# ahuang73/HemoCell

Hardware: AMD Instinct MI355X
Metric: MLUPS + cell-vertex updates/s, 256^3 pipeflow 10% Hct (higher is better)
Workload: dtype f64

## Files before the change

hemocell_amd/csrc/ibm.hip:

```cpp
#include "cells.h"
#include <type_traits>
#include <hipcub/hipcub.hpp>
#include <cstdlib>
#include <cstring>
#include <numeric>

namespace {

__global__ __launch_bounds__(256) void ibm_spread_kernel(LatView v, long n, const double *px, const double *py, const double *pz,
                                                         double *fx, double *fy, double *fz, const double *rx, const double *ry, const double *rz,
                                                         double *F, int limit_on, double f_limit, const int *vert_cell, const int *tag, const unsigned char *dead) {
  const long i = (long)blockIdx.x * 256 + threadIdx.x;
  if (i >= n) return;
  if (dead[i] || tag[vert_cell[i]] == 1) return;
  double f0 = fx[i], f1 = fy[i], f2 = fz[i];
  if (limit_on) {
    const double mag = sqrt((f0 * f0 + f1 * f1) + f2 * f2);
    if (mag > f_limit) {
      const double sc = f_limit / mag;
      f0 *= sc; f1 *= sc; f2 *= sc;
      fx[i] = f0; fy[i] = f1; fz[i] = f2;
    }
  }
  Stencil s;
  phi2_stencil(v, px[i], py[i], pz[i], s);
#pragma unroll
  for (int k = 0; k < 8; k++) {
    if (s.node[k] < 0) continue;
    v.dirty[s.node[k] >> 4] = v.epoch;
    double *Fn = F + 3 * s.node[k];
    unsafeAtomicAdd(Fn, ((rx ? rx[i] : 0.0) + f0) * s.w[k]);
    unsafeAtomicAdd(Fn + 1, ((ry ? ry[i] : 0.0) + f1) * s.w[k]);
    unsafeAtomicAdd(Fn + 2, ((rz ? rz[i] : 0.0) + f2) * s.w[k]);
  }
}

__global__ __launch_bounds__(256) void spread_emit_kernel(LatView v, int nv, long n, const int *order, long ebase, const double *px, const double *py,
                                                          const double *pz, double *fx, double *fy, double *fz, const double *rx, const double *ry,
                                                          const double *rz, int limit_on, double f_limit, const int *tag, const unsigned char *dead,
                                                          unsigned int *keys, int *vals, double *c0, double *c1, double *c2) {
  const long g = (long)blockIdx.x * 256 + threadIdx.x;
  if (g >= n) return;
  const int cell = order[g / nv];
  const long i = (long)cell * nv + (g % nv);
  const long e0 = (ebase + g) * 8;
  const bool live = tag[cell] != 1 && !dead[i];
  Stencil s;
  double f0 = 0.0, f1 = 0.0, f2 = 0.0;
  if (live) {
    f0 = fx[i]; f1 = fy[i]; f2 = fz[i];
    if (limit_on) {
      const double mag = sqrt((f0 * f0 + f1 * f1) + f2 * f2);
      if (mag > f_limit) { const double sc = f_limit / mag; f0 *= sc; f1 *= sc; f2 *= sc; fx[i] = f0; fy[i] = f1; fz[i] = f2; }
    }
    if (rx) { f0 = rx[i] + f0; f1 = ry[i] + f1; f2 = rz[i] + f2; }
    phi2_stencil(v, px[i], py[i], pz[i], s);
  }
#pragma unroll
  for (int k = 0; k < 8; k++) {
    const bool adm = live && s.node[k] >= 0;
    keys[e0 + k] = adm ? (unsigned int)s.node[k] : 0xffffffffu;
    vals[e0 + k] = (int)(e0 + k);
    c0[e0 + k] = adm ? f0 * s.w[k] : 0.0; c1[e0 + k] = adm ? f1 * s.w[k] : 0.0; c2[e0 + k] = adm ? f2 * s.w[k] : 0.0;
  }
}

__global__ __launch_bounds__(256) void spread_gather_kernel(LatView v, long n, const unsigned int *keys, const int *vals, const double *c0, const double *c1,
                                                            const double *c2, double *F) {
  const long s = (long)blockIdx.x * 256 + threadIdx.x;
  if (s >= n) return;
  const unsigned int key = keys[s];
  if (key == 0xffffffffu || (s > 0 && keys[s - 1] == key)) return;
  double a0 = 0.0, a1 = 0.0, a2 = 0.0;
  for (long q = s; q < n && keys[q] == key; q++) { const int e = vals[q]; a0 += c0[e]; a1 += c1[e]; a2 += c2[e]; }
  v.dirty[key >> 4] = v.epoch;
  double *Fn = F + 3 * (long)key;
  Fn[0] += a0; Fn[1] += a1; Fn[2] += a2;
}

struct PopView {
  const double *f; const double *F; double bx, by, bz; long qs;
  hc::BodyRegions reg;
};
struct OpenPopView : PopView { const int *ob_code; const double *ob_val; };
template <bool OPEN> using Pops = std::conditional_t<OPEN, OpenPopView, PopView>;

template <bool OPEN = false>
__device__ __forceinline__ void node_velocity(const LatView &v, const Pops<OPEN> &pv, int lx, int ly, int lz, long node, double u[3]) {
  if (v.halo_x && (lx <= -HALO || lx >= v.nx + HALO - 1)) { u[0] = u[1] = u[2] = 0.0; return; }
  if (v.halo_x && (lx == -1 || lx == v.nx)) {
    const double *hu = v.halo_u[lx < 0 ? 0 : 1];
    if (hu) { const long k = (long)ly * v.nz + lz; u[0] = hu[k]; u[1] = hu[v.ny_nz + k]; u[2] = hu[2L * v.ny_nz + k]; return; }
  }
  const hc::Nbr nb = hc::neighbours(v, v.plane, lx, ly, lz);
  double r = 0.0, jx = 0.0, jy = 0.0, jz = 0.0;
  [[maybe_unused]] double f[OPEN ? HC_Q : 1];
#define M(Q, CX, CY, CZ)                                                              \
  {                                                                                   \
    bool ok; const long off = hc::src_off<CX, CY, CZ>(nb, ok);                        \
    const double fq = ok ? pv.f[(long)Q * pv.qs + node + off] : 0.0;                 \
    if constexpr (OPEN) f[Q] = fq;                                                    \
    else {                                                                            \
      r += fq;                                                                        \
      if (CX == 1) jx += fq; else if (CX == -1) jx += -fq;                            \
      if (CY == 1) jy += fq; else if (CY == -1) jy += -fq;                            \
      if (CZ == 1) jz += fq; else if (CZ == -1) jz += -fq;                            \
    }                                                                                 \
  }
  FOR_Q(M)
#undef M
  if constexpr (OPEN) {
    if (v.mask[node] == 0) {
      const int code = pv.ob_code[node];
      if (code >= 0) hc::zou_he_node(f, code, pv.ob_val);
    }
    hc::moments(f, r, jx, jy, jz);
  }
  const double invRho = 1.0 / (1.0 + r);
  double bx = pv.bx, by = pv.by, bz = pv.bz;
  if (pv.reg.n) {
    int xg = v.x0 + lx;
    if (xg < 0) xg += v.nx_global; else if (xg >= v.nx_global) xg -= v.nx_global;
    region_force(pv.reg, xg, ly, lz, bx, by, bz);
  }
  u[0] = jx * invRho + (bx + pv.F[3 * node]) / 2.0;
  u[1] = jy * invRho + (by + pv.F[3 * node + 1]) / 2.0;
  u[2] = jz * invRho + (bz + pv.F[3 * node + 2]) / 2.0;
}

template <bool OPEN = false>
__global__ __launch_bounds__(256) void face_velocity_kernel(LatView v, Pops<OPEN> pv, int lx0, double *out0, int lx1, double *out1) {
  const int k = blockIdx.x * 256 + threadIdx.x;
  if (k >= v.ny_nz) return;
  const int lx = blockIdx.y ? lx1 : lx0;
  double *out = blockIdx.y ? out1 : out0;
  const int ly = k / v.nz, lz = k - ly * v.nz;
  const long node = (long)(lx + HALO) * v.plane + (long)ly * v.nz + lz;
  double u[3] = {0.0, 0.0, 0.0};
  if (v.mask[node] == 0) node_velocity<OPEN>(v, pv, lx, ly, lz, node, u);
  out[k] = u[0]; out[v.ny_nz + k] = u[1]; out[2L * v.ny_nz + k] = u[2];
}

template <bool OPEN = false>
__global__ __launch_bounds__(256) void ibm_interpolate_kernel(LatView v, Pops<OPEN> pv, long n, const double *px, const double *py,
                                                              const double *pz, double *vx, double *vy, double *vz, const int *vert_cell, const int *tag,
                                                              const unsigned char *dead) {
  const long i = (long)blockIdx.x * 256 + threadIdx.x;
  if (i >= n) return;
  if (dead[i] || tag[vert_cell[i]] == 1) return;
  Stencil s;
  phi2_stencil(v, px[i], py[i], pz[i], s);
  double a0 = 0.0, a1 = 0.0, a2 = 0.0;
#pragma unroll
  for (int k = 0; k < 8; k++) {
    if (s.node[k] < 0) continue;
    double u[3];
    node_velocity<OPEN>(v, pv, s.lx[k], s.ly[k], s.lz[k], s.node[k], u);
    a0 += (u[0] * s.w[k]); a1 += (u[1] * s.w[k]); a2 += (u[2] * s.w[k]);
  }
  vx[i] = a0; vy[i] = a1; vz[i] = a2;
}


constexpr int TILE_CAP = 5832;
constexpr int NODE_CAP = 1536;

struct Tile { int o[3]; int e[3]; int vol; int ow[3]; float r1, r2; };

__device__ __forceinline__ void tile_decode(const Tile &t, int i, int &tx, int &ty, int &tz) {
  const int q = (int)(((float)i + 0.5f) * t.r2);
  tz = i - q * t.e[2];
  tx = (int)(((float)q + 0.5f) * t.r1);
  ty = q - tx * t.e[1];
}

__device__ __forceinline__ int stencil_base(const LatView &v, double px, double py, double pz, int b[3]) {
  const double p[3] = {px, py, pz};
#pragma unroll
  for (int a = 0; a < 3; a++) { const long c = nearest_node(p[a]); b[a] = (int)c + ((p[a] < (double)c) ? -1 : 0); }
  return 0;
}

__device__ __forceinline__ long tile_node(const LatView &v, const Tile &t, int i, int &lx, int &ly, int &lz) {
  int tx, ty, tz;
  tile_decode(t, i, tx, ty, tz);
  lx = t.ow[0] + tx; ly = t.ow[1] + ty; lz = t.ow[2] + tz;
  if (v.wrap_x && lx >= v.nx) lx -= v.nx;
  if (v.per_y && ly >= v.ny) ly -= v.ny;
  if (v.per_z && lz >= v.nz) lz -= v.nz;
  return (long)(lx + HALO) * v.plane + ly * v.nz + lz;
}

__device__ __forceinline__ int xcd_contiguous(int b, int n) {
  const int per = n >> 3;
  const int main_n = per << 3;
  if (b >= main_n) return b;
  return (b & 7) * per + (b >> 3);
}

struct VStencil { double w[8]; int base; unsigned adm; };

constexpr int NVPT = 3;
constexpr int MAXW = 4;

#ifdef HC_IBM_PHASE_TIMES
__device__ unsigned long long g_phase[32];
#define PH_PARAM , long long &ph_last
#define PH_ARG , ph_last
#define PH_INIT long long ph_last = clock64();
#define STAMP(k) do { if (threadIdx.x == 0) { const long long ph_now = clock64(); atomicAdd(&g_phase[k], (unsigned long long)(ph_now - ph_last)); ph_last = ph_now; } } while (0)
#else
#define PH_PARAM
#define PH_ARG
#define PH_INIT
#define STAMP(k) do {} while (0)
#endif

__device__ __forceinline__ void block_bbox(int lo[3], int hi[3], int *s_red, Tile &t) {
  const int tid = threadIdx.x;
#pragma unroll
  for (int a = 0; a < 3; a++)
#pragma unroll
    for (int off = 32; off > 0; off >>= 1) { lo[a] = min(lo[a], __shfl_xor(lo[a], off)); hi[a] = max(hi[a], __shfl_xor(hi[a], off)); }
  if ((tid & 63) == 0) {
#pragma unroll
    for (int a = 0; a < 3; a++) { s_red[(tid >> 6) * 6 + a] = lo[a]; s_red[(tid >> 6) * 6 + 3 + a] = hi[a]; }
  }
  __syncthreads();
  const int nw = (blockDim.x + 63) >> 6;
#pragma unroll
  for (int a = 0; a < 3; a++) {
    int l = s_red[a], h = s_red[3 + a];
    for (int w = 1; w < nw; w++) { l = min(l, s_red[w * 6 + a]); h = max(h, s_red[w * 6 + 3 + a]); }
    t.o[a] = l; t.e[a] = h - l + 1;
  }
  const long vol = (long)t.e[0] * t.e[1] * t.e[2];
  t.vol = vol > 0x7fffffff ? 0x7fffffff : (int)vol;
}

__device__ __forceinline__ bool tile_finish(const LatView &v, Tile &t) {
  if (t.vol > TILE_CAP) return false;
  if ((v.wrap_x && t.e[0] > v.nx) || (v.per_y && t.e[1] > v.ny) || (v.per_z && t.e[2] > v.nz)) return false;
  t.ow[0] = v.wrap_x ? (int)pmod((long)t.o[0] - v.x0, v.nx) : t.o[0] - v.x0;
  t.ow[1] = v.per_y ? (int)pmod(t.o[1], v.ny) : t.o[1];
  t.ow[2] = v.per_z ? (int)pmod(t.o[2], v.nz) : t.o[2];
  t.r1 = 1.0f / (float)t.e[1]; t.r2 = 1.0f / (float)t.e[2];
  return true;
}

__device__ __forceinline__ unsigned char tile_mask(const LatView &v, const Tile &t, int i) {
  int tx, ty, tz;
  tile_decode(t, i, tx, ty, tz);
  int lx = t.ow[0] + tx, ly = t.ow[1] + ty, lz = t.ow[2] + tz;
  if (v.wrap_x) { if (lx >= v.nx) lx -= v.nx; }
  else if (v.halo_x) { if (lx < -HALO || lx >= v.nx + HALO) return 3; }
  else if (lx < 0 || lx >= v.nx) return 3;
  if (v.per_y) { if (ly >= v.ny) ly -= v.ny; } else if (ly < 0 || ly >= v.ny) return 3;
  if (v.per_z) { if (lz >= v.nz) lz -= v.nz; } else if (lz < 0 || lz >= v.nz) return 3;
  return v.mask[(long)(lx + HALO) * v.plane + ly * v.nz + lz];
}

__device__ __forceinline__ void tile_stencil(const Tile &t, const unsigned char *mt, double px, double py, double pz, const int b[3], VStencil &o) {
  const int sy = t.e[2], sx = t.e[1] * t.e[2];
  o.base = ((b[0] - t.o[0]) * t.e[1] + (b[1] - t.o[1])) * t.e[2] + (b[2] - t.o[2]);
  o.adm = 0;
  double total = 0.0;
#pragma unroll
  for (int i = 0; i < 2; i++)
#pragma unroll
    for (int j = 0; j < 2; j++)
#pragma unroll
      for (int k = 0; k < 2; k++) {
        const int idx = i * 4 + j * 2 + k;
        const double weight = phi2(px - (double)(b[0] + i)) * phi2(py - (double)(b[1] + j)) * phi2(pz - (double)(b[2] + k));
        const bool adm = (weight != 0.0) && (!mt || mt[o.base + i * sx + j * sy + k] == 0);
        if (adm) { total += weight; o.adm |= 1u << idx; }
        o.w[idx] = adm ? weight : 0.0;
      }
  const double coeff = 1.0 / total;
#pragma unroll
  for (int idx = 0; idx < 8; idx++) o.w[idx] *= coeff;
}

__device__ __forceinline__ bool tile_is_clear(const LatView &v, const Tile &t, int *s_near) {
  const int n[3] = {v.nx, v.ny, v.nz};
  bool inside = v.wallbrick != nullptr;
  int b0[3], nb[3];
#pragma unroll
  for (int a = 0; a < 3; a++) {
    const int lo = a == 0 ? t.ow[0] + HALO : t.ow[a], hi = lo + t.e[a] - 1, lim = a == 0 ? v.nx + 2 * HALO : n[a];
    inside = inside && lo >= 0 && hi < lim && (a != 0 || !v.wrap_x || (t.ow[0] >= 0 && t.ow[0] + t.e[0] <= v.nx));
    b0[a] = lo >> 3; nb[a] = (hi >> 3) - b0[a] + 1;
  }
  if (!inside) return false;
  if (nb[0] * nb[1] * nb[2] > 64) return false;
  if (threadIdx.x < 64) {
    const int l = threadIdx.x;
    bool near = false;
    if (l < nb[0] * nb[1] * nb[2]) {
      const int bz = l % nb[2], by = (l / nb[2]) % nb[1], bx = l / (nb[2] * nb[1]);
      near = v.wallbrick[((long)(b0[0] + bx) * v.nby + (b0[1] + by)) * v.nbz + (b0[2] + bz)] != 0;
    }
    const unsigned long long any = __ballot(near);
    if (l == 0) *s_near = any != 0ull;
  }
  __syncthreads();
  return *s_near == 0;
}

__device__ __forceinline__ bool cell_prologue(const LatView &v, int nv, long base, const double *px, const double *py, const double *pz,
                                              const unsigned char *dead, int *s_red, int *s_near, unsigned char *mt, Tile &t, VStencil vs[NVPT] PH_PARAM) {
  const int tid = threadIdx.x, nth = blockDim.x;
  double p[NVPT][3]; int b[NVPT][3]; bool live[NVPT];
  int lo[3] = {0x7fffffff, 0x7fffffff, 0x7fffffff}, hi[3] = {-0x7fffffff, -0x7fffffff, -0x7fffffff};
#pragma unroll
  for (int j = 0; j < NVPT; j++) {
    const int i = tid + j * nth;
    live[j] = i < nv && !(dead && dead[base + i]);
    if (live[j]) {
      p[j][0] = px[base + i]; p[j][1] = py[base + i]; p[j][2] = pz[base + i];
      stencil_base(v, p[j][0], p[j][1], p[j][2], b[j]);
#pragma unroll
      for (int a = 0; a < 3; a++) { lo[a] = min(lo[a], b[j][a]); hi[a] = max(hi[a], b[j][a] + 1); }
    }
  }
  block_bbox(lo, hi, s_red, t);
  STAMP(1);
  if (!tile_finish(v, t) || nv > NVPT * nth) return false;
  const bool clear = tile_is_clear(v, t, s_near);
  STAMP(2);
  if (!clear) {
#pragma unroll 4
    for (int i = tid; i < t.vol; i += nth) mt[i] = tile_mask(v, t, i);
    __syncthreads();
  }
  STAMP(3);
#pragma unroll
  for (int j = 0; j < NVPT; j++) {
    vs[j].adm = 0; vs[j].base = 0;
    if (live[j]) tile_stencil(t, clear ? nullptr : mt, p[j][0], p[j][1], p[j][2], b[j], vs[j]);
  }
  STAMP(4);
  return true;
}

constexpr unsigned short SLOT_FREE = 0xFFFF, SLOT_MARK = 0xFFFE;
__device__ __forceinline__ int compact_nodes(const Tile &t, const VStencil vs[NVPT], unsigned short *slot, unsigned short *list, int *s_count) {
  const int tid = threadIdx.x, nth = blockDim.x;
  const int sy = t.e[2], sx = t.e[1] * t.e[2];
  for (int i = tid; i < t.vol; i += nth) slot[i] = SLOT_FREE;
  if (tid == 0) *s_count = 0;
  __syncthreads();
#pragma unroll
  for (int j = 0; j < NVPT; j++)
#pragma unroll
    for (int k = 0; k < 8; k++) if (vs[j].adm & (1u << k)) slot[vs[j].base + (k >> 2) * sx + ((k >> 1) & 1) * sy + (k & 1)] = SLOT_MARK;
  __syncthreads();
  for (int i0 = 0; i0 < t.vol; i0 += nth) {
    const int i = i0 + tid;
    const bool marked = i < t.vol && slot[i] == SLOT_MARK;
    const unsigned long long b = __ballot(marked);
    int first = 0;
    if ((tid & 63) == 0 && b) first = atomicAdd(s_count, (int)__popcll(b));
    first = __shfl(first, 0);
    if (marked) {
      const int n = first + (int)__popcll(b & ((1ull << (tid & 63)) - 1ull));
      if (n < NODE_CAP) { slot[i] = (unsigned short)n; list[n] = (unsigned short)i; }
    }
  }
  __syncthreads();
  return *s_count;
}

__device__ void spread_direct(const LatView &v, int nv, long base, const double *px, const double *py, const double *pz, const double *fx,
                              const double *fy, const double *fz, const double *rx, const double *ry, const double *rz, double *F,
                              const unsigned char *dead) {
  for (int i = threadIdx.x; i < nv; i += blockDim.x) {
    if (dead && dead[base + i]) continue;
    Stencil s;
    phi2_stencil(v, px[base + i], py[base + i], pz[base + i], s);
    const double f0 = (rx ? rx[base + i] : 0.0) + fx[base + i], f1 = (ry ? ry[base + i] : 0.0) + fy[base + i], f2 = (rz ? rz[base + i] : 0.0) + fz[base + i];
#pragma unroll
    for (int k = 0; k < 8; k++) {
      if (s.node[k] < 0) continue;
      v.dirty[s.node[k] >> 4] = v.epoch;
      double *Fn = F + 3 * s.node[k];
      unsafeAtomicAdd(Fn, f0 * s.w[k]);
      unsafeAtomicAdd(Fn + 1, f1 * s.w[k]);
      unsafeAtomicAdd(Fn + 2, f2 * s.w[k]);
    }
  }
}

__global__ __launch_bounds__(256) void ibm_spread_cell_kernel(LatView v, int nv, const double *px, const double *py, const double *pz,
                                                              double *fx, double *fy, double *fz, const double *rx, const double *ry, const double *rz,
                                                              double *F, int limit_on, double f_limit, int xcd_ranges, const int *tag, const unsigned char *vdead) {
  __shared__ unsigned short slot[TILE_CAP];
  __shared__ __attribute__((aligned(16))) unsigned char raw[TILE_CAP > 2 * NODE_CAP ? TILE_CAP : 2 * NODE_CAP];
  unsigned char *mt = raw; unsigned short *list = reinterpret_cast<unsigned short *>(raw);
  __shared__ double acc[3 * NODE_CAP];
  __shared__ int s_red[6 * MAXW], s_count, s_near;
  const int tid = threadIdx.x, nth = blockDim.x;
  PH_INIT
  const int cell = xcd_ranges ? xcd_contiguous((int)blockIdx.x, (int)gridDim.x) : (int)blockIdx.x;
  const int state = tag[cell];
  if (state == 1) return;
  STAMP(0);
  const unsigned char *dead = state == 2 ? vdead : nullptr;
  const long base = (long)cell * nv;
  const bool in_regs = nv <= NVPT * nth;
  double f[NVPT][3];
  if (in_regs) {
#pragma unroll
    for (int j = 0; j < NVPT; j++) {
      const int i = tid + j * nth;
      f[j][0] = f[j][1] = f[j][2] = 0.0;
      if (i < nv) { f[j][0] = fx[base + i]; f[j][1] = fy[base + i]; f[j][2] = fz[base + i]; }
    }
  }
  Tile t; VStencil vs[NVPT];
  bool tiled = cell_prologue(v, nv, base, px, py, pz, dead, s_red, &s_near, mt, t, vs PH_ARG);
  if (limit_on) {
    if (in_regs) {
#pragma unroll
      for (int j = 0; j < NVPT; j++) {
        const int i = tid + j * nth;
        if (i < nv) {
          const double mag = sqrt((f[j][0] * f[j][0] + f[j][1] * f[j][1]) + f[j][2] * f[j][2]);
          if (mag > f_limit) { const double sc = f_limit / mag; f[j][0] *= sc; f[j][1] *= sc; f[j][2] *= sc; fx[base + i] = f[j][0]; fy[base + i] = f[j][1]; fz[base + i] = f[j][2]; }
        }
      }
    } else {
      for (int i = tid; i < nv; i += nth) {
        const double f0 = fx[base + i], f1 = fy[base + i], f2 = fz[base + i];
        const double mag = sqrt((f0 * f0 + f1 * f1) + f2 * f2);
        if (mag > f_limit) { const double sc = f_limit / mag; fx[base + i] = f0 * sc; fy[base + i] = f1 * sc; fz[base + i] = f2 * sc; }
      }
    }
  }
  const int n = tiled ? compact_nodes(t, vs, slot, list, &s_count) : 0;
  STAMP(5);
  if (!tiled || n > NODE_CAP) { spread_direct(v, nv, base, px, py, pz, fx, fy, fz, rx, ry, rz, F, dead); return; }
  const int sy = t.e[2], sx = t.e[1] * t.e[2];
  for (int k = tid; k < 3 * n; k += nth) acc[k] = 0.0;
  __syncthreads();
#pragma unroll
  for (int j = 0; j < NVPT; j++) {
    const int i = tid + j * nth;
    if (i >= nv || !vs[j].adm) continue;
    double fv[3];
    fv[0] = (rx ? rx[base + i] : 0.0) + f[j][0]; fv[1] = (ry ? ry[base + i] : 0.0) + f[j][1]; fv[2] = (rz ? rz[base + i] : 0.0) + f[j][2];
#pragma unroll
    for (int k = 0; k < 8; k++) {
      if (!(vs[j].adm & (1u << k))) continue;
      double *a = &acc[3 * slot[vs[j].base + (k >> 2) * sx + ((k >> 1) & 1) * sy + (k & 1)]];
      atomicAdd(a, fv[0] * vs[j].w[k]); atomicAdd(a + 1, fv[1] * vs[j].w[k]); atomicAdd(a + 2, fv[2] * vs[j].w[k]);
    }
  }
  __syncthreads();
  STAMP(6);
  for (int k = tid; k < 3 * n; k += nth) {
    const double val = acc[k];
    if (val != 0.0) {
      const int q = k / 3;
      int lx, ly, lz; const long node = tile_node(v, t, list[q], lx, ly, lz); v.dirty[node >> 4] = v.epoch;
      unsafeAtomicAdd(&F[3 * node + (k - 3 * q)], val);
    }
  }
  STAMP(7);
}

template <bool OPEN = false>
__global__ __launch_bounds__(256) void ibm_interpolate_cell_kernel(LatView v, Pops<OPEN> pv, int nv, const double *px, const double *py,
                                                                   const double *pz, double *vx, double *vy, double *vz, const int *slots, int xcd_ranges,
                                                                   const int *tag, const unsigned char *vdead) {
  __shared__ unsigned short slot[TILE_CAP];
  __shared__ __attribute__((aligned(16))) unsigned char raw[TILE_CAP > 2 * NODE_CAP ? TILE_CAP : 2 * NODE_CAP];
  unsigned char *mt = raw; unsigned short *list = reinterpret_cast<unsigned short *>(raw);
  __shared__ double ux[NODE_CAP], uy[NODE_CAP], uz[NODE_CAP];
  __shared__ int s_red[6 * MAXW], s_count, s_near;
  const int tid = threadIdx.x, nth = blockDim.x;
  const int cell = slots ? slots[blockIdx.x] : (xcd_ranges ? xcd_contiguous((int)blockIdx.x, (int)gridDim.x) : (int)blockIdx.x);
  const int state = tag[cell];
  if (state == 1) return;
  const unsigned char *dead = state == 2 ? vdead : nullptr;
  const long base = (long)cell * nv;
  Tile t; VStencil vs[NVPT];
  PH_INIT
  bool tiled = cell_prologue(v, nv, base, px, py, pz, dead, s_red, &s_near, mt, t, vs PH_ARG);
  const int sy = t.e[2], sx = t.e[1] * t.e[2];
  if (tiled) {
    if (compact_nodes(t, vs, slot, list, &s_count) > NODE_CAP) tiled = false;
    STAMP(12);
  }
  if (tiled) {
    const int n = s_count;
    for (int k = tid; k < n; k += nth) {
      int lx, ly, lz;
      const long node = tile_node(v, t, list[k], lx, ly, lz);
      double u[3];
      node_velocity<OPEN>(v, pv, lx, ly, lz, node, u);
      ux[k] = u[0]; uy[k] = u[1]; uz[k] = u[2];
    }
    __syncthreads();
    STAMP(13);
#pragma unroll
    for (int j = 0; j < NVPT; j++) {
      const int i = tid + j * nth;
      if (i >= nv) continue;
      double a0 = 0.0, a1 = 0.0, a2 = 0.0;
#pragma unroll
      for (int k = 0; k < 8; k++) {
        if (!(vs[j].adm & (1u << k))) continue;
        const int q = slot[vs[j].base + (k >> 2) * sx + ((k >> 1) & 1) * sy + (k & 1)];
        a0 += (ux[q] * vs[j].w[k]); a1 += (uy[q] * vs[j].w[k]); a2 += (uz[q] * vs[j].w[k]);
      }
      vx[base + i] = a0; vy[base + i] = a1; vz[base + i] = a2;
    }
    STAMP(14);
    return;
  }
  for (int i = tid; i < nv; i += nth) {
    if (dead && dead[base + i]) continue;
    Stencil s;
    phi2_stencil(v, px[base + i], py[base + i], pz[base + i], s);
    double a0 = 0.0, a1 = 0.0, a2 = 0.0;
#pragma unroll
    for (int k = 0; k < 8; k++) {
      if (s.node[k] < 0) continue;
      double u[3];
      node_velocity<OPEN>(v, pv, s.lx[k], s.ly[k], s.lz[k], s.node[k], u);
      a0 += (u[0] * s.w[k]); a1 += (u[1] * s.w[k]); a2 += (u[2] * s.w[k]);
    }
    vx[base + i] = a0; vy[base + i] = a1; vz[base + i] = a2;
  }
}

PopView make_pops(const hc_lattice *L) {
  return PopView{L->f[L->cur], L->force[(L->fcur + 2) % 3], L->body[0], L->body[1], L->body[2], (long)L->qstride, L->regions};
}
OpenPopView open_of(const hc_lattice *L, const PopView &pv) {
  OpenPopView o;
  static_cast<PopView &>(o) = pv;
  o.ob_code = L->ob_code; o.ob_val = L->ob_val;
  return o;
}

}

#define HC_LAUNCH_POPS(K, grid, block, v, pv, ...)                                                                      \
  hc::launch_open(L, pv, [&](auto open, const auto &pops) {                                                             \
    hipLaunchKernelGGL(K<decltype(open)::value>, grid, block, 0, hc::stream(), v, pops, __VA_ARGS__);                   \
  })

static int g_ibm_per_vertex = 0;
extern "C" int hc_debug_ibm_per_vertex(int on) { g_ibm_per_vertex = on; return HC_OK; }
static int g_reproducible = -1;
static bool reproducible() {
  if (g_reproducible < 0) { const char *e = std::getenv("HEMOCELL_REPRODUCIBLE_SPREAD"); g_reproducible = (e && *e && *e != '0') ? 1 : 0; }
  return g_reproducible == 1;
}
extern "C" int hc_set_reproducible_spread(int on) { g_reproducible = on ? 1 : 0; return HC_OK; }

static int spread_reproducible(hc_cells *C, int force_limit) {
  const LatView v = make_view(C->L);
  HC_REQUIRE(v.npad * 3 < 0xffffffffL && C->nverts * 8 < 0x7fffffffL, "reproducible spread: lattice or vertex count beyond its 32-bit keys");
  const long n_e = C->nverts * 8;
  int rc;
  if (n_e > C->det_cap) {
    HC_HIP(hipDeviceSynchronize());
    const long cap = n_e + n_e / 4 + 4096;
    C->det_cap = 0;
    for (int k = 0; k < 2; k++) if ((rc = C->det_keys[k].reserve((size_t)cap)) != HC_OK || (rc = C->det_vals[k].reserve((size_t)cap)) != HC_OK) return rc;
    for (int k = 0; k < 3; k++) if ((rc = C->det_val[k].reserve((size_t)cap)) != HC_OK) return rc;
    size_t tmp_bytes = 0;
    HC_HIP(hipcub::DeviceRadixSort::SortPairs(nullptr, tmp_bytes, C->det_keys[0].p, C->det_keys[1].p, C->det_vals[0].p, C->det_vals[1].p, (int)cap, 0, 32, hc::stream()));
    if ((rc = C->det_tmp.reserve(tmp_bytes)) != HC_OK) return rc;
    C->det_cap = cap;
  }
  std::vector<int> order((size_t)0);
  std::vector<long> obase((size_t)C->ntypes, 0);
  for (int t = 0; t < C->ntypes; t++) {
    const size_t nc = (size_t)C->ncells[t], o = order.size();
    obase[(size_t)t] = (long)o;
    order.resize(o + nc);
    std::iota(order.begin() + (long)o, order.end(), 0);
    const std::vector<long> &ids = C->hids[t];
    std::stable_sort(order.begin() + (long)o, order.end(), [&](int a, int b) { return ids[(size_t)a] < ids[(size_t)b]; });
  }
  int *d_order = nullptr;
  rc = stage_ints(C, 2, &d_order, order.data(), (int)order.size()); if (rc != HC_OK) return rc;
  long ebase = 0;
  for (int t = 0; t < C->ntypes; t++) {
    const int nv = C->types[t]->host.nv;
    const long n = C->ncells[t] * nv;
    if (n == 0) continue;
    const TypeArrays a = vert_arrays(C, t);
    hipLaunchKernelGGL(spread_emit_kernel, dim3((unsigned)((n + 255) / 256)), dim3(256), 0, hc::stream(), v, nv, n, (const int *)(d_order + obase[(size_t)t]), ebase,
                       a.p[0], a.p[1], a.p[2], a.f[0], a.f[1], a.f[2], a.r[0], a.r[1], a.r[2], force_limit, C->P.f_limit, a.tag, a.dead, C->det_keys[0], C->det_vals[0],
                       C->det_val[0], C->det_val[1], C->det_val[2]);
    HC_HIP(hipGetLastError());
    ebase += n;
  }
  int bits = 1;
  while (bits < 32 && (1L << bits) <= v.npad) bits++;
  size_t tmp = C->det_tmp.cap;
  HC_HIP(hipcub::DeviceRadixSort::SortPairs(C->det_tmp.p, tmp, C->det_keys[0].p, C->det_keys[1].p, C->det_vals[0].p, C->det_vals[1].p, (int)n_e, 0, bits, hc::stream()));
  hipLaunchKernelGGL(spread_gather_kernel, dim3((unsigned)((n_e + 255) / 256)), dim3(256), 0, hc::stream(), v, n_e, (const unsigned int *)C->det_keys[1],
                     (const int *)C->det_vals[1], (const double *)C->det_val[0], (const double *)C->det_val[1], (const double *)C->det_val[2], C->L->force[C->L->fcur]);
  HC_HIP(hipGetLastError());
  return HC_OK;
}
#ifdef HC_IBM_PHASE_TIMES
extern "C" int hc_debug_phase_times(double *out) {
  unsigned long long h[32];
  if (hipMemcpyFromSymbol(h, HIP_SYMBOL(g_phase), sizeof(h)) != hipSuccess) return HC_ERR_HIP;
  for (int k = 0; k < 32; k++) out[k] = (double)h[k];
  std::memset(h, 0, sizeof(h));
  if (hipMemcpyToSymbol(HIP_SYMBOL(g_phase), h, sizeof(h)) != hipSuccess) return HC_ERR_HIP;
  return HC_OK;
}
#endif

extern "C" {

int hcp_spread(hc_cells *C, int force_limit) {
  HC_REQUIRE(C, "hcp_spread: null pointer");
  int rc = sync_to_device(C); if (rc != HC_OK) return rc;
  if (C->nverts == 0) return HC_OK;
  hc::ProfScope prof(hc::PK_SPREAD);
  if (reproducible()) return spread_reproducible(C, force_limit);
  const LatView v = make_view(C->L);
  for (int t = 0; t < C->ntypes; t++) {
    const long n = C->ncells[t] * C->types[t]->host.nv;
    if (n == 0) continue;
    const int nv = C->types[t]->host.nv;
    const TypeArrays a = vert_arrays(C, t);
    if (g_ibm_per_vertex)
      hipLaunchKernelGGL(ibm_spread_kernel, dim3((unsigned)((n + 255) / 256)), dim3(256), 0, hc::stream(), v, n, a.p[0], a.p[1], a.p[2], a.f[0], a.f[1], a.f[2],
                         a.r[0], a.r[1], a.r[2], C->L->force[C->L->fcur], force_limit, C->P.f_limit, a.vert_cell, a.tag_all, a.dead);
    else
      hipLaunchKernelGGL(ibm_spread_cell_kernel, dim3((unsigned)C->ncells[t]), dim3(nv > 128 ? 256 : 128), 0, hc::stream(), v, nv, a.p[0], a.p[1], a.p[2],
                         a.f[0], a.f[1], a.f[2], a.r[0], a.r[1], a.r[2], C->L->force[C->L->fcur], force_limit, C->P.f_limit, 1, a.tag, a.dead);
    HC_HIP(hipGetLastError());
  }
  return HC_OK;
}

int hcp_interpolate(hc_cells *C) {
  HC_REQUIRE(C, "hcp_interpolate: null pointer");
  int rc = sync_to_device(C); if (rc != HC_OK) return rc;
  if (C->nverts == 0) return HC_OK;
  hc::ProfScope prof(hc::PK_INTERP);
  const hc_lattice *L = C->L;
  const LatView v = make_view(L);
  const PopView pv = make_pops(L);
  for (int t = 0; t < C->ntypes; t++) {
    const long n = C->ncells[t] * C->types[t]->host.nv;
    if (n == 0) continue;
    const int nv = C->types[t]->host.nv;
    const TypeArrays a = vert_arrays(C, t);
    if (g_ibm_per_vertex)
      HC_LAUNCH_POPS(ibm_interpolate_kernel, dim3((unsigned)((n + 255) / 256)), dim3(256), v, pv, n, a.p[0], a.p[1], a.p[2], a.v[0], a.v[1], a.v[2],
                     a.vert_cell, a.tag_all, a.dead);
    else
      HC_LAUNCH_POPS(ibm_interpolate_cell_kernel, dim3((unsigned)C->ncells[t]), dim3(nv > 128 ? 256 : 128), v, pv, nv, a.p[0], a.p[1], a.p[2], a.v[0], a.v[1], a.v[2],
                     (const int *)nullptr, 1, a.tag, a.dead);
    HC_HIP(hipGetLastError());
  }
  return HC_OK;
}

int hcl_face_velocity_pack(hc_lattice *L, int side, double *dev_buf) {
  HC_REQUIRE(L && dev_buf && (side == 0 || side == 1), "hcl_face_velocity_pack: bad arguments");
  LatView v = make_view(L);
  v.halo_u[0] = v.halo_u[1] = nullptr;
  const PopView pv = make_pops(L);
  HC_LAUNCH_POPS(face_velocity_kernel, dim3((unsigned)((L->plane + 255) / 256), 1, 1), dim3(256), v, pv, side == 0 ? 0 : L->nx - 1, dev_buf, 0, (double *)nullptr);
  HC_HIP(hipGetLastError());
  return HC_OK;
}
int hcl_face_velocity_pack_both(hc_lattice *L, double *dev_lo, double *dev_hi) {
  HC_REQUIRE(L, "hcl_face_velocity_pack_both: null lattice");
  if (!dev_lo && !dev_hi) return HC_OK;
  if (!dev_lo || !dev_hi) return hcl_face_velocity_pack(L, dev_lo ? 0 : 1, dev_lo ? dev_lo : dev_hi);
  LatView v = make_view(L);
  v.halo_u[0] = v.halo_u[1] = nullptr;
  const PopView pv = make_pops(L);
  HC_LAUNCH_POPS(face_velocity_kernel, dim3((unsigned)((L->plane + 255) / 256), 2, 1), dim3(256), v, pv, 0, dev_lo, L->nx - 1, dev_hi);
  HC_HIP(hipGetLastError());
  return HC_OK;
}

int hcl_download_face_velocity(hc_lattice *L, int side, double *host_u) {
  HC_REQUIRE(L && host_u && (side == 0 || side == 1), "hcl_download_face_velocity: bad arguments");
  hc::DevBuf<double> d;
  int rc = d.reserve(3 * L->plane); if (rc != HC_OK) return rc;
  rc = hcl_face_velocity_pack(L, side, d);
  if (rc == HC_OK && hipMemcpyAsync(host_u, d, 3 * L->plane * sizeof(double), hipMemcpyDeviceToHost, hc::stream()) != hipSuccess) { hc::set_error("hcl_download_face_velocity: copy failed"); rc = HC_ERR_HIP; }
  if (rc == HC_OK && hipStreamSynchronize(hc::stream()) != hipSuccess) { hc::set_error("hcl_download_face_velocity: synchronise failed"); rc = HC_ERR_HIP; }
  return rc;
}

int hcp_interpolate_cells(hc_cells *C, int type, const int *slots, int n) { return hcc::interpolate_cells_staged(C, type, slots, n, 1); }

}

int hcc::interpolate_cells_staged(hc_cells *C, int type, const int *slots, int n, int which) {
  HC_REQUIRE(C && type >= 0 && type < C->ntypes && n >= 0 && which >= 0 && which < 19, "hcp_interpolate_cells: bad arguments");
  if (n == 0) return HC_OK;
  HC_REQUIRE(slots, "hcp_interpolate_cells: null pointer");
  int rc = sync_to_device(C); if (rc != HC_OK) return rc;
  for (int i = 0; i < n; i++) HC_REQUIRE(slots[i] >= 0 && slots[i] < C->ncells[type], "hcp_interpolate_cells: slot out of range");
  int *d_slots = nullptr;
  rc = stage_ints(C, which, &d_slots, slots, n); if (rc != HC_OK) return rc;
  hc::ProfScope prof(hc::PK_INTERP);
  const hc_lattice *L = C->L;
  const LatView v = make_view(L);
  const PopView pv = make_pops(L);
  const TypeArrays a = vert_arrays(C, type);
  const int nv = C->types[type]->host.nv;
  HC_LAUNCH_POPS(ibm_interpolate_cell_kernel, dim3((unsigned)n), dim3(nv > 128 ? 256 : 128), v, pv, nv, a.p[0], a.p[1], a.p[2], a.v[0], a.v[1], a.v[2],
                 (const int *)d_slots, 0, a.tag, a.dead);
  HC_HIP(hipGetLastError());
  return HC_OK;
}
```

Measured before the change: 15830.

## Compact tile nodes with shared bitmask and wave prefix scan, issue position loads before tag check

Node compaction in the per-cell spread and interpolate kernels now marks touched tile nodes in a 256-word shared bitmap with atomicOr, instead of initialising and marking a full ushort slot array. Slots are then assigned with a single-wave prefix scan over popcounts plus readlane, which removes the slot-array init pass and the per-wave atomicAdd on a shared counter. The bitmap is aliased into the acc and ux shared buffers, so zeroing acc up front also clears it, and vertex position loads are issued before the cell tag is read to hide latency. The aliasing is subtle: acc zeroing, the marks region and ux reuse must not overlap live data, and the scan relies on a single 64-lane wave covering the whole tile.

Measured after the change: 15900, median of 5. No clear change (+0.5%).

```diff
diff --git a/hemocell_amd/csrc/ibm.hip b/hemocell_amd/csrc/ibm.hip
--- a/hemocell_amd/csrc/ibm.hip
+++ b/hemocell_amd/csrc/ibm.hip
@@ -308,17 +308,29 @@
   return *s_near == 0;
 }
 
-__device__ __forceinline__ bool cell_prologue(const LatView &v, int nv, long base, const double *px, const double *py, const double *pz,
-                                              const unsigned char *dead, int *s_red, int *s_near, unsigned char *mt, Tile &t, VStencil vs[NVPT] PH_PARAM) {
+enum { CELL_GONE = 0, CELL_UNTILED = 1, CELL_TILED = 2 };
+__device__ __forceinline__ int cell_prologue(const LatView &v, int nv, int cell, const int *tag, const unsigned char *vdead, const double *px, const double *py,
+                                             const double *pz, const unsigned char *&dead, int *s_red, int *s_near, unsigned char *mt, Tile &t,
+                                             VStencil vs[NVPT] PH_PARAM) {
   const int tid = threadIdx.x, nth = blockDim.x;
+  const long base = (long)cell * nv;
   double p[NVPT][3]; int b[NVPT][3]; bool live[NVPT];
   int lo[3] = {0x7fffffff, 0x7fffffff, 0x7fffffff}, hi[3] = {-0x7fffffff, -0x7fffffff, -0x7fffffff};
+#pragma unroll
+  for (int j = 0; j < NVPT; j++) {
+    const int i = tid + j * nth;
+    p[j][0] = p[j][1] = p[j][2] = 0.0;
+    if (i < nv) { p[j][0] = px[base + i]; p[j][1] = py[base + i]; p[j][2] = pz[base + i]; }
+  }
+  const int state = tag[cell];
+  if (state == 1) return CELL_GONE;
+  STAMP(0);
+  dead = state == 2 ? vdead : nullptr;
 #pragma unroll
   for (int j = 0; j < NVPT; j++) {
     const int i = tid + j * nth;
     live[j] = i < nv && !(dead && dead[base + i]);
     if (live[j]) {
-      p[j][0] = px[base + i]; p[j][1] = py[base + i]; p[j][2] = pz[base + i];
       stencil_base(v, p[j][0], p[j][1], p[j][2], b[j]);
 #pragma unroll
       for (int a = 0; a < 3; a++) { lo[a] = min(lo[a], b[j][a]); hi[a] = max(hi[a], b[j][a] + 1); }
@@ -326,7 +338,7 @@
   }
   block_bbox(lo, hi, s_red, t);
   STAMP(1);
-  if (!tile_finish(v, t) || nv > NVPT * nth) return false;
+  if (!tile_finish(v, t) || nv > NVPT * nth) return CELL_UNTILED;
   const bool clear = tile_is_clear(v, t, s_near);
   STAMP(2);
   if (!clear) {
@@ -341,35 +353,52 @@
     if (live[j]) tile_stencil(t, clear ? nullptr : mt, p[j][0], p[j][1], p[j][2], b[j], vs[j]);
   }
   STAMP(4);
-  return true;
-}
-
-constexpr unsigned short SLOT_FREE = 0xFFFF, SLOT_MARK = 0xFFFE;
-__device__ __forceinline__ int compact_nodes(const Tile &t, const VStencil vs[NVPT], unsigned short *slot, unsigned short *list, int *s_count) {
-  const int tid = threadIdx.x, nth = blockDim.x;
+  return CELL_TILED;
+}
+
+constexpr int MARK_WORDS = 256;
+static_assert(MARK_WORDS * 32 >= TILE_CAP && MARK_WORDS == 64 * 4, "one 16-byte read per lane covers the tile");
+__device__ __forceinline__ void clear_marks(unsigned *marks) {
+  for (int i = threadIdx.x; i < MARK_WORDS; i += blockDim.x) marks[i] = 0u;
+}
+__device__ __forceinline__ unsigned long long wave_read(unsigned long long x, int src) {
+  const unsigned lo = (unsigned)__builtin_amdgcn_readlane((int)(unsigned)x, src), hi = (unsigned)__builtin_amdgcn_readlane((int)(unsigned)(x >> 32), src);
+  return (unsigned long long)lo | ((unsigned long long)hi << 32);
+}
+__device__ __forceinline__ int compact_nodes(const Tile &t, const VStencil vs[NVPT], unsigned *marks, unsigned short *slot, unsigned short *list) {
+  const int tid = threadIdx.x, lane = tid & 63;
   const int sy = t.e[2], sx = t.e[1] * t.e[2];
-  for (int i = tid; i < t.vol; i += nth) slot[i] = SLOT_FREE;
-  if (tid == 0) *s_count = 0;
+#pragma unroll
+  for (int j = 0; j < NVPT; j++)
+#pragma unroll
+    for (int k2 = 0; k2 < 4; k2++) {
+      const unsigned m2 = (vs[j].adm >> (2 * k2)) & 3u;
+      if (!m2) continue;
+      const int e = vs[j].base + (k2 >> 1) * sx + (k2 & 1) * sy;
+      const unsigned long long mm = (unsigned long long)m2 << (e & 31);
+      if ((unsigned)mm) atomicOr(&marks[e >> 5], (unsigned)mm);
+      if ((unsigned)(mm >> 32)) atomicOr(&marks[(e >> 5) + 1], (unsigned)(mm >> 32));
+    }
   __syncthreads();
-#pragma unroll
-  for (int j = 0; j < NVPT; j++)
-#pragma unroll
-    for (int k = 0; k < 8; k++) if (vs[j].adm & (1u << k)) slot[vs[j].base + (k >> 2) * sx + ((k >> 1) & 1) * sy + (k & 1)] = SLOT_MARK;
+  const uint4 m = reinterpret_cast<const uint4 *>(marks)[lane];
+  const unsigned long long b0 = (unsigned long long)m.x | ((unsigned long long)m.y << 32), b1 = (unsigned long long)m.z | ((unsigned long long)m.w << 32);
+  const int c0 = (int)__popcll(b0), c1 = (int)__popcll(b1);
+  int incl = c0 + c1;
+#pragma unroll
+  for (int off = 1; off < 64; off <<= 1) { const int o = __shfl_up(incl, off); if (lane >= off) incl += o; }
+  const int n = __shfl(incl, 63);
+  const int p0 = incl - c0 - c1;
+  const int nw = (int)blockDim.x >> 6;
+  for (int r = __builtin_amdgcn_readfirstlane(tid >> 6); 64 * r < t.vol; r += nw) {
+    unsigned long long b = wave_read(b0, r >> 1);
+    int first = __builtin_amdgcn_readlane(p0, r >> 1);
+    if (r & 1) { first += (int)__popcll(b); b = wave_read(b1, r >> 1); }
+    if (!((b >> lane) & 1ull)) continue;
+    const int q = first + (int)__popcll(b & ((1ull << lane) - 1ull));
+    if (q < NODE_CAP) { slot[64 * r + lane] = (unsigned short)q; list[q] = (unsigned short)(64 * r + lane); }
+  }
   __syncthreads();
-  for (int i0 = 0; i0 < t.vol; i0 += nth) {
-    const int i = i0 + tid;
-    const bool marked = i < t.vol && slot[i] == SLOT_MARK;
-    const unsigned long long b = __ballot(marked);
-    int first = 0;
-    if ((tid & 63) == 0 && b) first = atomicAdd(s_count, (int)__popcll(b));
-    first = __shfl(first, 0);
-    if (marked) {
-      const int n = first + (int)__popcll(b & ((1ull << (tid & 63)) - 1ull));
-      if (n < NODE_CAP) { slot[i] = (unsigned short)n; list[n] = (unsigned short)i; }
-    }
-  }
-  __syncthreads();
-  return *s_count;
+  return n;
 }
 
 __device__ void spread_direct(const LatView &v, int nv, long base, const double *px, const double *py, const double *pz, const double *fx,
@@ -398,15 +427,14 @@
   __shared__ unsigned short slot[TILE_CAP];
   __shared__ __attribute__((aligned(16))) unsigned char raw[TILE_CAP > 2 * NODE_CAP ? TILE_CAP : 2 * NODE_CAP];
   unsigned char *mt = raw; unsigned short *list = reinterpret_cast<unsigned short *>(raw);
-  __shared__ double acc[3 * NODE_CAP];
-  __shared__ int s_red[6 * MAXW], s_count, s_near;
+  __shared__ __attribute__((aligned(16))) double acc[3 * NODE_CAP];
+  constexpr int ACC_FREE = 3 * NODE_CAP - MARK_WORDS / 2;
+  unsigned *marks = reinterpret_cast<unsigned *>(acc + ACC_FREE);
+  static_assert(ACC_FREE > 0 && ACC_FREE % 2 == 0, "the bit map is 16-byte aligned");
+  __shared__ int s_red[6 * MAXW], s_near;
   const int tid = threadIdx.x, nth = blockDim.x;
   PH_INIT
   const int cell = xcd_ranges ? xcd_contiguous((int)blockIdx.x, (int)gridDim.x) : (int)blockIdx.x;
-  const int state = tag[cell];
-  if (state == 1) return;
-  STAMP(0);
-  const unsigned char *dead = state == 2 ? vdead : nullptr;
   const long base = (long)cell * nv;
   const bool in_regs = nv <= NVPT * nth;
   double f[NVPT][3];
@@ -418,8 +446,13 @@
       if (i < nv) { f[j][0] = fx[base + i]; f[j][1] = fy[base + i]; f[j][2] = fz[base + i]; }
     }
   }
+  for (int k = tid; k < 3 * NODE_CAP / 2; k += nth) reinterpret_cast<double2 *>(acc)[k] = double2{0.0, 0.0};
+  static_assert(sizeof(unsigned) * MARK_WORDS == sizeof(double) * (3 * NODE_CAP - ACC_FREE), "zeroing acc clears the bit map (clear_marks)");
   Tile t; VStencil vs[NVPT];
-  bool tiled = cell_prologue(v, nv, base, px, py, pz, dead, s_red, &s_near, mt, t, vs PH_ARG);
+  const unsigned char *dead = nullptr;
+  const int found = cell_prologue(v, nv, cell, tag, vdead, px, py, pz, dead, s_red, &s_near, mt, t, vs PH_ARG);
+  if (found == CELL_GONE) return;
+  const bool tiled = found == CELL_TILED;
   if (limit_on) {
     if (in_regs) {
 #pragma unroll
@@ -438,12 +471,14 @@
       }
     }
   }
-  const int n = tiled ? compact_nodes(t, vs, slot, list, &s_count) : 0;
+  const int n = tiled ? compact_nodes(t, vs, marks, slot, list) : 0;
   STAMP(5);
   if (!tiled || n > NODE_CAP) { spread_direct(v, nv, base, px, py, pz, fx, fy, fz, rx, ry, rz, F, dead); return; }
   const int sy = t.e[2], sx = t.e[1] * t.e[2];
-  for (int k = tid; k < 3 * n; k += nth) acc[k] = 0.0;
-  __syncthreads();
+  if (3 * n > ACC_FREE) {
+    for (int k = ACC_FREE + tid; k < 3 * n; k += nth) acc[k] = 0.0;
+    __syncthreads();
+  }
 #pragma unroll
   for (int j = 0; j < NVPT; j++) {
     const int i = tid + j * nth;
@@ -477,24 +512,28 @@
   __shared__ unsigned short slot[TILE_CAP];
   __shared__ __attribute__((aligned(16))) unsigned char raw[TILE_CAP > 2 * NODE_CAP ? TILE_CAP : 2 * NODE_CAP];
   unsigned char *mt = raw; unsigned short *list = reinterpret_cast<unsigned short *>(raw);
-  __shared__ double ux[NODE_CAP], uy[NODE_CAP], uz[NODE_CAP];
-  __shared__ int s_red[6 * MAXW], s_count, s_near;
+  __shared__ __attribute__((aligned(16))) double ux[NODE_CAP];
+  __shared__ double uy[NODE_CAP], uz[NODE_CAP];
+  unsigned *marks = reinterpret_cast<unsigned *>(ux);
+  __shared__ int s_red[6 * MAXW], s_near;
   const int tid = threadIdx.x, nth = blockDim.x;
   const int cell = slots ? slots[blockIdx.x] : (xcd_ranges ? xcd_contiguous((int)blockIdx.x, (int)gridDim.x) : (int)blockIdx.x);
-  const int state = tag[cell];
-  if (state == 1) return;
-  const unsigned char *dead = state == 2 ? vdead : nullptr;
   const long base = (long)cell * nv;
   Tile t; VStencil vs[NVPT];
   PH_INIT
-  bool tiled = cell_prologue(v, nv, base, px, py, pz, dead, s_red, &s_near, mt, t, vs PH_ARG);
+  clear_marks(marks);
+  const unsigned char *dead = nullptr;
+  const int found = cell_prologue(v, nv, cell, tag, vdead, px, py, pz, dead, s_red, &s_near, mt, t, vs PH_ARG);
+  if (found == CELL_GONE) return;
+  bool tiled = found == CELL_TILED;
   const int sy = t.e[2], sx = t.e[1] * t.e[2];
+  int n = 0;
   if (tiled) {
-    if (compact_nodes(t, vs, slot, list, &s_count) > NODE_CAP) tiled = false;
+    n = compact_nodes(t, vs, marks, slot, list);
+    if (n > NODE_CAP) tiled = false;
     STAMP(12);
   }
   if (tiled) {
-    const int n = s_count;
     for (int k = tid; k < n; k += nth) {
       int lx, ly, lz;
       const long node = tile_node(v, t, list[k], lx, ly, lz);
```
